# lhoyer/improving_segmentation_with_selfsupervised_depth

Hardware: AMD Instinct MI355X
Metric: train images/sec, ResNet-101 joint seg+depth @512x1024 (higher is better)
Workload: dtype f32

## Files before the change

### improving_segmentation_with_selfsupervised_depth_amd/csrc/conv_igemm.hip

```cpp
#include <type_traits>
#include "segsde_common.h"
#include "conv_small.h"
#include "winograd.h"
#include <cstdlib>
#include <mutex>
#include <cstring>

namespace {

struct ConvP {
  const float* x0; const float* x1; const float* w; const float* bias;
  float* y; float* y2;
  int B, H, W, C0, C1, ld0, ld1, up0;
  int Ho, Wo, N, ldy, ldy2, nsplit;
  int KH, KW, stride, dil, pad, pad_mode, in_div;
  int Ctot, Ktot, M, act, sum2x2;
  int vecout;
  int nb, ne;
  const float* zero;
  int kh0, khs, kw0, kws, KWf, Kfull, os, oph, opw, OHf, OWf;
  double* stats;
  int accum;
  const float* agy; int agld, agkind;
  unsigned mg1, mg2; int sf1, sf2, d1, d2;
// ... 1621 lines not shown
    return (b.ne - b.nb <= 32) ? launch_igemm<128, 32, 4, 1>(b, s) : launch_igemm<128, 64, 2, 2>(b, s);
  }
  return launch_igemm<128, 128, 2, 2>(q, s);
}

__global__ __launch_bounds__(256) void adjoint_corner_kernel(const float* dy, int lddy, const float* wd , float* y, int ldy,
                                                             float* y2, int ldy2, int nsplit, int B, int H, int W, int N, int C,
                                                             const float* agy, int agld, int agkind, int accumulate_only) {
  const int total = B * 4 * N;
  for (int e = blockIdx.x * 256 + threadIdx.x; e < total; e += gridDim.x * 256) {
    const int n = e % N, t = e / N, k = t & 3, b = t >> 2;
    const int bot = k >> 1, rgt = k & 1;
    const int i = bot ? H - 2 : 1, j = rgt ? W - 2 : 1, r = bot ? H - 1 : 0, sc = rgt ? W - 1 : 0;
    const int tap = (bot ? 0 : 2) * 3 + (rgt ? 0 : 2);
    const float* dp = dy + ((long)(b * H + r) * W + sc) * lddy;
    const float* wp = wd + ((long)n * 9 + tap) * C;
    float acc = 0.f;
    for (int c = 0; c < C; ++c) acc += dp[c] * wp[c];
    const long pix = (long)(b * H + i) * W + j;
    if (agy && n < nsplit) acc *= segsde_act_grad_from_out(agy[pix * agld + n], agkind);
    if (n < nsplit) y[pix * ldy + n] += acc; else y2[pix * ldy2 + (n - nsplit)] += acc;
  }
}

int launch_adjoint_by_borders(const ConvP& p, hipStream_t s, bool with_main = true) {
  ConvP q = p;
  q.pad_mode = SEGSDE_PAD_ZERO;
  ConvP bl[4];
  for (int k = 0; k < 4; ++k) {
    const bool rowl = k < 2, far = k & 1;
    ConvP b = p;
    b.pad_mode = SEGSDE_PAD_ZERO;
    b.KH = rowl ? 1 : 3; b.KW = rowl ? 3 : 1;
    b.Ho = rowl ? 1 : p.H; b.Wo = rowl ? p.W : 1; b.M = p.B * b.Ho * b.Wo;
    b.pad = rowl ? (far ? -(p.H - 1) : 0) : 1;
    b.padw = rowl ? 1 : (far ? -(p.W - 1) : 0);
    b.Ktot = 3 * p.Ctot; b.Kfull = p.Kfull; b.KWf = b.KW;
    b.wtap = rowl ? p.Ctot : 3 * p.Ctot;
    const int tap0 = rowl ? (far ? 0 : 6) : (far ? 0 : 2);
    b.w = p.w + (long)tap0 * p.Ctot;
    b.kh0 = 0; b.khs = 1; b.kw0 = 0; b.kws = 1;
    b.submap = 1; b.os = 1; b.OHf = p.H; b.OWf = p.W;
    b.oph = rowl ? (far ? p.H - 2 : 1) : 0; b.opw = rowl ? 0 : (far ? p.W - 2 : 1);
    b.osfast = (rowl && p.W % 128 == 0) ? 1 : 0;
    b.accum = 1; b.lin = 0; b.stats = nullptr; b.bias = nullptr; b.act = 0;
    set_divs(b);
    if (!igemm_fast_ok(b) || !b.vecout) return SEGSDE_ERR_UNSUPPORTED;
    bl[k] = b;
  }
  if (with_main)
    if (int e = launch_by_n(q, s)) return e;
  for (int k = 0; k < 4; ++k)
    if (int e = launch_by_n(bl[k], s)) return e;
  if (probing()) return 0;
  hipLaunchKernelGGL(adjoint_corner_kernel, dim3(segsde_cdiv((long)p.B * 4 * p.N, 256)), dim3(256), 0, s, p.x0, p.ld0, p.w, p.y, p.ldy,
                     p.y2, p.ldy2, p.nsplit, p.B, p.H, p.W, p.N, p.Ctot, p.agy, p.agld, p.agkind, 0);
  SEGSDE_CHECK_LAUNCH();
  return 0;
}
bool adjoint_by_borders_ok(const ConvP& p) {
  const bool big = (long)p.B * p.H * p.W >= (1L << 21) || p.cmp;
  return big && p.pad_mode == SEGSDE_PAD_REFLECT_ADJOINT && igemm_fast_ok(p) && !p.sum2x2 && p.vecout && p.H >= 4 &&
         p.W >= 4 && p.C1 == 0 && p.KH == 3 && p.KW == 3 && p.nb == 0 && p.ne == p.N;
}
}

namespace {
int borders_params(const segsde_conv_desc* d, const float* dy, const float* wdpack, float* y, const float* act_out, int act_ld,
                   int act_kind, ConvP& p) {
  if (int e = validate(d)) return e;
  if (d->pad_mode != SEGSDE_PAD_REFLECT_ADJOINT || d->C1 || d->up0 || d->sum2x2 || d->in_div > 1 || d->act != 0) return SEGSDE_ERR_UNSUPPORTED;
  p = make_params(d, dy, nullptr, wdpack, nullptr, y, nullptr);
  if (act_out) {
    if (act_kind < SEGSDE_ACT_RELU || act_kind > SEGSDE_ACT_SIGMOID || act_ld < p.nsplit || (act_ld % 4) || !aligned16(act_out))
      return SEGSDE_ERR_UNSUPPORTED;
    p.agy = act_out; p.agld = act_ld; p.agkind = act_kind;
  }
  if (!(igemm_fast_ok(p) && p.vecout && p.H >= 4 && p.W >= 4 && p.KH == 3 && p.KW == 3 && p.nb == 0 && p.ne == p.N))
    return SEGSDE_ERR_UNSUPPORTED;
  return 0;
}
}

extern "C" int segsde_reflect_adjoint_borders_ok(const segsde_conv_desc* d, int act_ld) {
  ConvP p;
  float* fake = reinterpret_cast<float*>(16);
  return borders_params(d, fake, fake, fake, act_ld ? fake : nullptr, act_ld, SEGSDE_ACT_ELU, p) == 0;
}

extern "C" int segsde_reflect_adjoint_borders(const segsde_conv_desc* d, const float* dy, const float* wdpack, float* y,
                                              const float* act_out, int act_ld, int act_kind, void* stream) {
  if (!dy || !wdpack || !y) return SEGSDE_ERR_NULL;
  ConvP p;
  if (int e = borders_params(d, dy, wdpack, y, act_out, act_ld, act_kind, p)) return e;
  return launch_adjoint_by_borders(p, static_cast<hipStream_t>(stream), false);
}

extern "C" long segsde_conv2d_stats_rows(const segsde_conv_desc* d) {
  if (validate(d)) return 0;
  float dummy[4];
  const ConvP p = make_params(d, dummy, dummy, dummy, nullptr, reinterpret_cast<float*>(16), nullptr);
  return stats_rows(d, p);
}

extern "C" int segsde_conv2d_forward(const segsde_conv_desc* d, const float* x0, const float* x1, const float* wpack,
                                     const float* bias, float* y, float* y2, void* stream) {
  return segsde_conv2d_forward_stats(d, x0, x1, wpack, bias, y, y2, nullptr, stream);
}

extern "C" int segsde_conv2d_forward_stats(const segsde_conv_desc* d, const float* x0, const float* x1, const float* wpack,
                                           const float* bias, float* y, float* y2, double* stats, void* stream) {
  return segsde_conv2d_dgrad_actgrad(d, x0, x1, wpack, bias, y, y2, stats, nullptr, 0, 0, stream);
}

extern "C" int segsde_conv2d_dgrad_actgrad(const segsde_conv_desc* d, const float* x0, const float* x1, const float* wpack,
                                           const float* bias, float* y, float* y2, double* stats, const float* act_out,
                                           int act_ld, int act_kind, void* stream) {
  if (int e = validate(d)) return e;
  if (!x0 || !wpack || !y || (d->C1 && !x1)) return SEGSDE_ERR_NULL;
  ConvP p = make_params(d, x0, x1, wpack, bias, y, y2);
  if (act_out) {
    if (stats || bias || d->act != 0 || act_kind < SEGSDE_ACT_RELU || act_kind > SEGSDE_ACT_SIGMOID || act_ld < p.nsplit ||
        (act_ld % 4) || !aligned16(act_out) || d->in_div > 1)
      return SEGSDE_ERR_UNSUPPORTED;
    p.agy = act_out; p.agld = act_ld; p.agkind = act_kind;
  }
  if (stats) {
    if (stats_rows(d, p) == 0) return SEGSDE_ERR_UNSUPPORTED;
    p.stats = stats;
  }
  const bool parity_split = d->in_div == 2 && d->stride == 1 && (d->dil & 1) && d->pad_mode == SEGSDE_PAD_ZERO && !d->sum2x2 &&
                            d->C1 == 0 && !d->up0 && !bias && d->act == 0 && !y2 && p.vecout;
  if (d->accumulate) {
    if (y2 || bias || d->act != 0 || d->sum2x2 || (d->in_div > 1 && !parity_split) || !p.vecout || d->Cout == 1 || d->C0 % 4 != 0 ||
        d->C0 == 1 || (d->pad_mode == SEGSDE_PAD_REFLECT_ADJOINT && !igemm_fast_ok(p)))
      return SEGSDE_ERR_UNSUPPORTED;
  }
  hipStream_t s = static_cast<hipStream_t>(stream);
  const bool plain3x3 = d->KH == 3 && d->KW == 3 && d->stride == 1 && d->dil == 1 && d->pad == 1 && d->C1 == 0 && !d->up0 &&
                        d->in_div <= 1 && !d->sum2x2 && d->H == d->Ho && d->W == d->Wo;
  if (plain3x3 && d->Cout == 1 && d->pad_mode != SEGSDE_PAD_REFLECT_ADJOINT && segsde_c1_supported(d->C0, d->ld0) &&
      aligned16(x0) && aligned16(wpack))
    return probing() ? 0 : segsde_c1_forward(x0, d->ld0, d->B, d->H, d->W, d->C0, wpack, bias, d->pad_mode == SEGSDE_PAD_REFLECT, d->act, y,
                             d->ldy, stream);
  if (plain3x3 && d->C0 == 1 && d->pad_mode != SEGSDE_PAD_REFLECT && !bias && d->act == 0 &&
      segsde_c1_supported(d->Cout, p.ldy) && p.vecout)
    return probing() ? 0 : segsde_c1_dgrad(x0, d->ld0, d->B, d->H, d->W, d->Cout, wpack, d->pad_mode == SEGSDE_PAD_REFLECT_ADJOINT, y, p.ldy,
                           y2, p.ldy2, p.nsplit, p.agy, p.agld, p.agkind, stream);
  const bool plain1x1 = d->KH == 1 && d->KW == 1 && d->stride == 1 && d->pad == 0 && d->C1 == 0 && !d->up0 && d->in_div <= 1 &&
                        !d->sum2x2 && d->H == d->Ho && d->W == d->Wo;
  if (plain1x1 && !stats && !p.agy && d->C0 % 4 != 0 && d->ld0 == d->C0 && aligned16(x0) && !bias && d->act == 0 && !y2 &&
      segsde_skinny_supported(d->C0, d->Cout) && p.vecout)
    return probing() ? 0 : segsde_skinny_nk(x0, d->C0, wpack, (long)d->B * d->H * d->W, d->Cout, y, p.ldy, stream);
  if (parity_split) {
    bool ok = true;
    ConvP sub[4]; int nsub = 0; bool empty = false;
    for (int ph = 0; ph < 2 && ok; ++ph)
      for (int pw = 0; pw < 2 && ok; ++pw) {
        ConvP q = p;
        int kh0 = -1, kw0 = -1;
        for (int k = 0; k < d->KH; ++k) if (((ph + k * d->dil - d->pad) & 1) == 0) { kh0 = k; break; }
        for (int k = 0; k < d->KW; ++k) if (((pw + k * d->dil - d->pad) & 1) == 0) { kw0 = k; break; }
        const int nI = (d->Ho - ph + 1) / 2, nJ = (d->Wo - pw + 1) / 2;
        if (nI <= 0 || nJ <= 0) continue;
        if (kh0 < 0 || kw0 < 0) { empty = true; continue; }
        q.kh0 = kh0; q.khs = 2; q.kw0 = kw0; q.kws = 2; q.KWf = d->KW; q.Kfull = p.Ktot;
        q.KH = (d->KH - kh0 + 1) / 2; q.KW = (d->KW - kw0 + 1) / 2;
        q.Ktot = q.KH * q.KW * q.Ctot;
        q.in_div = 1;
        q.pad = -((ph + kh0 * d->dil - d->pad) / 2);
        q.padw = -((pw + kw0 * d->dil - d->pad) / 2);
        q.os = 2; q.submap = 1; q.oph = ph; q.opw = pw; q.OHf = d->Ho; q.OWf = d->Wo;
        q.Ho = nI; q.Wo = nJ; q.M = d->B * nI * nJ;
        set_divs(q);
        if (!igemm_fast_ok(q)) ok = false;
        sub[nsub++] = q;
      }
    if (!ok && d->accumulate) return SEGSDE_ERR_UNSUPPORTED;
    if (ok) {
      if (empty && !d->accumulate && !probing()) {
        if (hipMemsetAsync(y, 0, (size_t)d->B * d->Ho * d->Wo * p.ldy * sizeof(float), s) != hipSuccess) return SEGSDE_ERR_SHAPE;
      }
      for (int i = 0; i < nsub; ++i) {
        const ConvP& q = sub[i];
        int e;
        if (q.N <= 32) e = launch_igemm<128, 32, 4, 1>(q, s);
        else if (q.N <= 64) e = launch_igemm<128, 64, 2, 2>(q, s);
        else e = launch_igemm<128, 128, 2, 2>(q, s);
        if (e) return e;
      }
      return 0;
    }
  }
  if (p.agy && d->pad_mode == SEGSDE_PAD_REFLECT_ADJOINT && !igemm_fast_ok(p))
    return SEGSDE_ERR_UNSUPPORTED;
  if (d->sum2x2) {
    if ((d->Ho & 1) || (d->Wo & 1) || d->stride != 1 || d->act != 0 || bias) return SEGSDE_ERR_SHAPE;
    if (!igemm_fast_ok(p)) return SEGSDE_ERR_UNSUPPORTED;
  }
  if (adjoint_by_borders_ok(p)) {
    const int e = launch_adjoint_by_borders(p, s);
    if (e != SEGSDE_ERR_UNSUPPORTED) return e;
  }
  if (int e = launch_by_n(p, s)) return e;
  if (d->pad_mode == SEGSDE_PAD_REFLECT_ADJOINT && !igemm_fast_ok(p))
    return launch_reflect_fix(x0, p.ld0, wpack, y, p.ldy, y2, p.ldy2, p.nsplit, p.B, p.H, p.W, p.N, p.C0, s);
  return 0;
}

namespace {
template <int BKT, int BN, int WM, int WN, int MODE, int CMP = 0>
int launch_wgrad_mode(const ConvP& p, const float* dy, int lddy, float* ws, int splits, int cps, hipStream_t stream) {
  const dim3 grid(segsde_cdiv(p.Ktot, BKT) * segsde_cdiv(p.N, BN) * splits);
  size_t smem = 2 * (size_t)BP * (BKT + BN) * sizeof(float);
  if (MODE == 5)
    smem += 2 * (size_t)((p.Ho - 1) * p.stride + (p.KH - 1) * p.dil + 1 + (p.Wo - 1) * p.stride + (p.KW - 1) * p.dil + 1) * sizeof(unsigned);
  auto k = conv_wgrad_kernel<BKT, BN, WM, WN, MODE, CMP>;
  (void)hipFuncSetAttribute(reinterpret_cast<const void*>(k), hipFuncAttributeMaxDynamicSharedMemorySize, (int)smem);
  hipLaunchKernelGGL(k, grid, dim3(256), smem, stream, p, dy, lddy, ws, cps);
  SEGSDE_CHECK_LAUNCH();
  return 0;
}

int wgrad_mode(const ConvP& p, const float* dy, int lddy) {
  const bool vec = vec_ok(p) && (p.N % 4 == 0) && (lddy % 4 == 0) && aligned16(dy);
  const long e0 = (long)p.B * (p.H >> p.up0) * (p.W >> p.up0) * p.ld0, e1 = (long)p.B * p.H * p.W * p.ld1;
  const bool fast = vec_ok(p) && e0 < (1L << 31) && e1 < (1L << 31);
  const long i0 = (long)(p.H >> p.up0) * (p.W >> p.up0) * p.ld0 * 4, i1 = (long)p.H * p.W * p.ld1 * 4;
  const bool table = p.Wo % BP == 0 && i0 <= (1L << 30) && i1 <= (1L << 30) && (long)BP * p.os * lddy * 4 < (1L << 30);
  if (fast && vec && table) return 5;
  if (fast) return 3;
  return vec ? 1 : 0;
}

int wgrad_compute(const ConvP& p, const float* dy, int lddy) { return wgrad_mode(p, dy, lddy) == 5 ? p.cmp : 0; }

template <int BKT, int BN, int WM, int WN>
int launch_wgrad(const ConvP& p, const float* dy, int lddy, float* ws, int splits, int cps, hipStream_t stream) {
  const int cmp = wgrad_compute(p, dy, lddy);
  if (probing()) return probe_note(cmp);
  switch (wgrad_mode(p, dy, lddy)) {
    case 5:
      return cmp == 1   ? launch_wgrad_mode<BKT, BN, WM, WN, 5, 1>(p, dy, lddy, ws, splits, cps, stream)
             : cmp == 2 ? launch_wgrad_mode<BKT, BN, WM, WN, 5, 2>(p, dy, lddy, ws, splits, cps, stream)
                        : launch_wgrad_mode<BKT, BN, WM, WN, 5, 0>(p, dy, lddy, ws, splits, cps, stream);
    case 3: return launch_wgrad_mode<BKT, BN, WM, WN, 3>(p, dy, lddy, ws, splits, cps, stream);
    case 1: return launch_wgrad_mode<BKT, BN, WM, WN, 1>(p, dy, lddy, ws, splits, cps, stream);
    default: return launch_wgrad_mode<BKT, BN, WM, WN, 0>(p, dy, lddy, ws, splits, cps, stream);
  }
}

void wgrad_plan(const segsde_conv_desc* d, int& bkt, int& bn, int& splits, int& cps) {
  const int Ktot = d->KH * d->KW * (d->C0 + d->C1);
  const long M = (long)d->B * d->Ho * d->Wo;
  bn = d->Cout <= 32 ? 32 : (d->Cout <= 64 ? 64 : 128);
  bkt = 128;
  const long tiles = (long)segsde_cdiv(Ktot, bkt) * segsde_cdiv(d->Cout, bn);
  const int nchunks = segsde_cdiv(M, BP);
  const long slots = 256L * (bn == 128 ? 2 : 3);
  constexpr long WG_OVERHEAD_CHUNKS = 4;
  long best = -1, best_cost = 0;
  const long smax = nchunks / 8 > 1 ? (nchunks / 8 < 1024 ? nchunks / 8 : 1024) : 1;
  for (long sp = 1; sp <= smax; ++sp) {
    const long c = (nchunks + sp - 1) / sp, se = (nchunks + c - 1) / c;
    const long waves = (tiles * se + slots - 1) / slots;
    const long cost = waves * (c + WG_OVERHEAD_CHUNKS);
    if (best < 0 || cost < best_cost) { best = se; best_cost = cost; }
  }
  cps = segsde_cdiv(nchunks, best);
  splits = segsde_cdiv(nchunks, cps);
}
}

namespace {
bool c1_wgrad_route(const segsde_conv_desc* d) {
  return d->Cout == 1 && d->KH == 3 && d->KW == 3 && d->stride == 1 && d->dil == 1 && d->pad == 1 && d->C1 == 0 && !d->up0 &&
         d->H == d->Ho && d->W == d->Wo && d->pad_mode != SEGSDE_PAD_REFLECT_ADJOINT && segsde_c1_supported(d->C0, d->ld0);
}
}

extern "C" size_t segsde_conv2d_wgrad_workspace(const segsde_conv_desc* d) {
  if (validate(d)) return 0;
  if (c1_wgrad_route(d)) return segsde_c1_wgrad_workspace(d->C0);
  int bkt, bn, splits, cps;
  wgrad_plan(d, bkt, bn, splits, cps);
  return (size_t)splits * d->KH * d->KW * (d->C0 + d->C1) * d->Cout * sizeof(float);
}

extern "C" int segsde_conv2d_wgrad(const segsde_conv_desc* d, const float* x0, const float* x1, const float* dy,
                                   int lddy, float* dw_oihw, float* workspace, size_t workspace_bytes, void* stream) {
  if (int e = validate(d)) return e;
  if (!x0 || !dy || !dw_oihw || !workspace || (d->C1 && !x1)) return SEGSDE_ERR_NULL;
  if (workspace_bytes < segsde_conv2d_wgrad_workspace(d)) return SEGSDE_ERR_WORKSPACE;
  if (c1_wgrad_route(d) && aligned16(x0))
    return probing() ? 0 : segsde_c1_wgrad(x0, d->ld0, d->B, d->H, d->W, d->C0, dy, lddy, d->pad_mode == SEGSDE_PAD_REFLECT, dw_oihw, workspace,
                           stream);
  ConvP p = make_params(d, x0, x1, dy , nullptr, workspace, nullptr);
  hipStream_t s = static_cast<hipStream_t>(stream);
  int bkt, bn, splits, cps;
  wgrad_plan(d, bkt, bn, splits, cps);
  int e;
  if (bn == 32) e = launch_wgrad<128, 32, 4, 1>(p, dy, lddy, workspace, splits, cps, s);
  else if (bn == 64) e = launch_wgrad<128, 64, 2, 2>(p, dy, lddy, workspace, splits, cps, s);
  else e = launch_wgrad<128, 128, 2, 2>(p, dy, lddy, workspace, splits, cps, s);
  if (e) return e;
  if (probing()) return 0;
  const long total = (long)p.Ktot * p.N;
  hipLaunchKernelGGL(wgrad_reduce_kernel, dim3(segsde_cdiv(total, 32)), dim3(256), 1024, s, workspace, splits,
                     p.Ktot, p.N, p.Ctot, d->KH * d->KW, (wgrad_mode(p, dy, lddy) == 5 && p.C1 > 0) ? p.C0 : 0, dw_oihw, p.Ctot, 0);
  SEGSDE_CHECK_LAUNCH();
  return 0;
}

namespace {
__device__ __host__ inline int upfold_th(int py, int kh) { return py == 0 ? (kh == 0 ? 0 : 1) : (kh == 2 ? 1 : 0); }

__global__ __launch_bounds__(256) void upfold_pack_kernel(const float* w, int Cout, int C0, int Ctot, float* wf, float* wd) {
  const long total = 4L * Cout * 4 * C0;
  for (long e = blockIdx.x * 256L + threadIdx.x; e < total; e += (long)gridDim.x * 256) {
    const int c = (int)(e % C0); long t = e / C0;
    const int tw = (int)(t & 1), th = (int)((t >> 1) & 1); t >>= 2;
    const int n = (int)(t % Cout), cls = (int)(t / Cout);
    const int py = cls >> 1, px = cls & 1;
    const float* wp = w + ((long)n * Ctot + c) * 9;
    float sum = 0.f;
    for (int kh = 0; kh < 3; ++kh) {
      if (upfold_th(py, kh) != th) continue;
      float r = 0.f;
      for (int kw = 0; kw < 3; ++kw)
        if (upfold_th(px, kw) == tw) r += wp[kh * 3 + kw];
      sum += r;
    }
    wf[e] = sum;
    const int a = 3 - 2 * th - py, b = 3 - 2 * tw - px;
    wd[(((long)c * 4 + a) * 4 + b) * Cout + n] = sum;
  }
}

__global__ __launch_bounds__(256) void upfold_dgrad_fix_kernel(const float* dy, int lddy, const float* wf, float* dx, int lddx,
                                                               int B, int H2, int W2, int C0, int Cout, const float* agy,
                                                               int agld, int agkind) {
  const int nbord = H2 >= 2 ? 2 * W2 + 2 * (H2 - 2) : W2;
  const long total = (long)B * nbord * C0;
  const int H = 2 * H2, W = 2 * W2;
  for (long e = blockIdx.x * 256L + threadIdx.x; e < total; e += (long)gridDim.x * 256) {
    const int c = (int)(e % C0); long t = e / C0;
    const int q = (int)(t % nbord), b = (int)(t / nbord);
    int i, j;
    if (q < W2) { i = 0; j = q; }
    else if (q < 2 * W2) { i = H2 - 1; j = q - W2; }
    else { const int r = q - 2 * W2; i = 1 + (r >> 1); j = (r & 1) ? W2 - 1 : 0; }
    float acc = 0.f;
    for (int a = 0; a < 4; ++a) {
      const int rm = 2 * i - 1 + a;
      const int rx = (i == 0 && a == 3) ? 0 : ((i == H2 - 1 && a == 0) ? H - 1 : -1);
      const int py = (a & 1) ? 0 : 1, th = a >= 2 ? 0 : 1;
      for (int bb = 0; bb < 4; ++bb) {
        const int cm = 2 * j - 1 + bb;
        const int cx = (j == 0 && bb == 3) ? 0 : ((j == W2 - 1 && bb == 0) ? W - 1 : -1);
        if (rx < 0 && cx < 0) continue;
        const int px = (bb & 1) ? 0 : 1, tw = bb >= 2 ? 0 : 1;
        const float* wrow = wf + (((long)(py * 2 + px) * Cout) * 4 + th * 2 + tw) * C0 + c;
        for (int v = 0; v < 3; ++v) {
          const int r = v == 1 ? rm : rx, sc = v == 0 ? cm : cx;
          if (r < 0 || r >= H || sc < 0 || sc >= W) continue;
          const float* dp = dy + ((long)(b * H + r) * W + sc) * lddy;
          float part = 0.f;
          for (int n = 0; n < Cout; ++n) part += dp[n] * wrow[(long)n * 4 * C0];
          acc += part;
        }
      }
    }
    const long pix = (long)(b * H2 + i) * W2 + j;
    if (agy) acc *= segsde_act_grad_from_out(agy[pix * agld + c], agkind);
    dx[pix * lddx + c] += acc;
  }
}

__global__ __launch_bounds__(256) void upfold_dgrad_corner_kernel(const float* dy, int lddy, const float* wdfold, float* dx, int lddx,
                                                                  int B, int H2, int W2, int C0, int Cout, const float* agy,
                                                                  int agld, int agkind) {
  const int total = B * 4 * C0;
  const int H = 2 * H2, W = 2 * W2;
  for (int e = blockIdx.x * 256 + threadIdx.x; e < total; e += gridDim.x * 256) {
    const int c = e % C0, t = e / C0, k = t & 3, b = t >> 2;
    const int bot = k >> 1, rgt = k & 1;
    const int i = bot ? H2 - 1 : 0, j = rgt ? W2 - 1 : 0, r = bot ? H - 1 : 0, sc = rgt ? W - 1 : 0;
    const int a = bot ? 0 : 3, bb = rgt ? 0 : 3;
    const float* dp = dy + ((long)(b * H + r) * W + sc) * lddy;
    const float* wp = wdfold + (((long)c * 4 + a) * 4 + bb) * Cout;
    float acc = 0.f;
    for (int n = 0; n < Cout; ++n) acc += dp[n] * wp[n];
    const long pix = (long)(b * H2 + i) * W2 + j;
    if (agy) acc *= segsde_act_grad_from_out(agy[pix * agld + c], agkind);
    dx[pix * lddx + c] += acc;
  }
}

__global__ __launch_bounds__(256) void upfold_wgrad_reduce_kernel(const float* part, int splits, int C0, int N, float* dw,
                                                                  int CtotDst) {
  SEGSDE_SMEM;
  float* sh = reinterpret_cast<float*>(segsde_smem);
  const long total = (long)N * C0 * 9;
  const long slab = 4L * C0 * N;
  const int tx = threadIdx.x & 31, ty = threadIdx.x >> 5;
  const long e = blockIdx.x * 32L + tx;
  float acc = 0.f;
  int n = 0, tap = 0, c = 0;
  if (e < total) {
    n = (int)(e % N); const long t = e / N;
    tap = (int)(t % 9); c = (int)(t / 9);
    const int kh = tap / 3, kw = tap - kh * 3;
    for (int cls = 0; cls < 4; ++cls) {
      const int th = upfold_th(cls >> 1, kh), tw = upfold_th(cls & 1, kw);
      const float* src = part + (long)cls * splits * slab + ((long)(th * 2 + tw) * C0 + c) * N + n;
      float s0 = 0.f, s1 = 0.f;
      int z = ty;
      for (; z + 8 < splits; z += 16) { s0 += src[(long)z * slab]; s1 += src[(long)(z + 8) * slab]; }
      if (z < splits) s0 += src[(long)z * slab];
      acc += s0 + s1;
    }
  }
  sh[ty * 32 + tx] = acc;
  __syncthreads();
  if (ty == 0 && e < total) {
    float s = 0.f;
    for (int j = 0; j < 8; ++j) s += sh[j * 32 + tx];
    dw[((long)n * CtotDst + c) * 9 + tap] = s;
  }
}

bool upfold_shape_ok(const segsde_conv_desc* d) {
  return d->up0 && d->KH == 3 && d->KW == 3 && d->stride == 1 && d->dil == 1 && d->pad == 1 && d->pad_mode == SEGSDE_PAD_REFLECT &&
         d->H == d->Ho && d->W == d->Wo && !(d->H & 1) && !(d->W & 1) && d->H >= 4 && d->W >= 4 && d->C0 % 32 == 0 &&
         d->C1 % 32 == 0 && d->Cout % 4 == 0 && d->in_div <= 1 && !d->sum2x2 && !d->accumulate;
}

ConvP upfold_class_fwd(const segsde_conv_desc* d, const float* x0, const float* wf, const float* bias, float* y, int py, int px) {
  segsde_conv_desc c = *d;
  c.H = d->H / 2; c.W = d->W / 2; c.Ho = c.H; c.Wo = c.W; c.up0 = 0; c.C1 = 0; c.ld1 = 0; c.KH = 2; c.KW = 2;
  c.pad = 1 - py; c.pad_mode = SEGSDE_PAD_ZERO; c.nsplit = 0; c.ldy2 = 0;
  if (d->C1) c.act = 0;
  ConvP q = make_params(&c, x0, nullptr, wf + (long)(py * 2 + px) * d->Cout * 4 * d->C0, d->C1 ? nullptr : bias, y, nullptr);
  q.pad_mode = SEGSDE_PAD_CLAMP_; q.padw = 1 - px;
  q.os = 2; q.submap = 1; q.oph = py; q.opw = px; q.OHf = d->H; q.OWf = d->W;
  q.osfast = (c.Wo % 128 == 0) ? 1 : 0;
  q.lin = 0;
  return q;
}
// ... 545 lines not shown
```

### improving_segmentation_with_selfsupervised_depth_amd/csrc/conv_small.h

```cpp
#pragma once
#include <stddef.h>
bool segsde_c1_supported(int C, int ldx);
size_t segsde_c1_wgrad_workspace(int C);
int segsde_c1_forward(const float* x, int ldx, int B, int H, int W, int C, const float* wpack, const float* bias, int reflect,
                      int act, float* y, int ldy, void* stream);
int segsde_c1_dgrad(const float* dz, int lddz, int B, int H, int W, int C, const float* wdpack, int adjoint, float* dx, int lddx,
                    float* dx2, int lddx2, int nsplit, const float* agy, int agld, int agkind, void* stream);
int segsde_c1_wgrad(const float* x, int ldx, int B, int H, int W, int C, const float* dz, int lddz, int reflect, float* dw,
                    float* workspace, void* stream);
bool segsde_skinny_supported(int K, int C);
int segsde_skinny_nk(const float* a, int K, const float* w, long M, int C, float* y, int ldy, void* stream);
```

### improving_segmentation_with_selfsupervised_depth_amd/csrc/conv_small.hip

```cpp
#include "segsde_common.h"
#include "conv_small.h"

namespace {
#define ST(s) static_cast<hipStream_t>(s)

__device__ __forceinline__ int refl1(int i, int n) { return i < 0 ? -i : (i >= n ? 2 * n - 2 - i : i); }

template <int LP>
__global__ __launch_bounds__(256) void c1_fwd_kernel(const float* x, int ldx, int B, int H, int W, const float* wp ,
                                                     const float* bias, int reflect, int act, float* y, int ldy) {
  constexpr int PPB = 256 / LP;
  const int lane_c = threadIdx.x % LP, slot = threadIdx.x / LP;
  float4 w[9];
#pragma unroll
  for (int t = 0; t < 9; ++t) w[t] = *reinterpret_cast<const float4*>(wp + t * (LP * 4) + 4 * lane_c);
  const float b0 = bias ? bias[0] : 0.f;
  const long npix = (long)B * H * W;
  for (long p0 = (long)blockIdx.x * PPB; p0 < npix; p0 += (long)gridDim.x * PPB) {
    const long p = p0 + slot;
    const bool live = p < npix;
    const long pp = live ? p : 0;
    const int wq = (int)(pp % W); const long t2 = pp / W; const int hq = (int)(t2 % H); const long b = t2 / H;
    float acc = 0.f;
#pragma unroll
    for (int kh = 0; kh < 3; ++kh) {
      int hi = hq + kh - 1; bool okh = true;
      if (reflect) hi = refl1(hi, H); else okh = (unsigned)hi < (unsigned)H;
#pragma unroll
      for (int kw = 0; kw < 3; ++kw) {
        int wi = wq + kw - 1; bool ok = okh;
        if (reflect) wi = refl1(wi, W); else ok = ok && (unsigned)wi < (unsigned)W;
        if (ok) {
          const float4 v = *reinterpret_cast<const float4*>(x + ((b * H + hi) * W + wi) * ldx + 4 * lane_c);
          const float4 ww = w[kh * 3 + kw];
          acc += v.x * ww.x + v.y * ww.y + v.z * ww.z + v.w * ww.w;
        }
      }
    }
#pragma unroll
    for (int o = LP / 2; o > 0; o >>= 1) acc += __shfl_xor(acc, o);
    if (lane_c == 0 && live) y[p * ldy] = segsde_act(acc + b0, act);
  }
}

template <int LP>
__global__ __launch_bounds__(256) void c1_dgrad_kernel(const float* dz, int lddz, int B, int H, int W,
                                                       const float* wd , int adjoint, float* dx, int lddx,
                                                       float* dx2, int lddx2, int nsplit, const float* agy, int agld,
                                                       int agkind) {
  constexpr int PPB = 256 / LP;
  const int lane_c = threadIdx.x % LP, slot = threadIdx.x / LP;
  float w[4][9];
#pragma unroll
  for (int j = 0; j < 4; ++j)
#pragma unroll
    for (int t = 0; t < 9; ++t) w[j][t] = wd[(4 * lane_c + j) * 9 + t];
  const long npix = (long)B * H * W;
  for (long p0 = (long)blockIdx.x * PPB; p0 < npix; p0 += (long)gridDim.x * PPB) {
    const long p = p0 + slot;
    if (p >= npix) continue;
    const int wq = (int)(p % W); const long t2 = p / W; const int hq = (int)(t2 % H); const long b = t2 / H;
    float a0 = 0.f, a1 = 0.f, a2 = 0.f, a3 = 0.f;
    int hp[3], wpp[3], nh = 0, nw = 0;
    hp[nh++] = hq; wpp[nw++] = wq;
    if (adjoint) {
      if (hq == 1) hp[nh++] = -1;
      if (hq == H - 2) hp[nh++] = H;
      if (wq == 1) wpp[nw++] = -1;
      if (wq == W - 2) wpp[nw++] = W;
    }
    for (int a = 0; a < nh; ++a)
      for (int bb = 0; bb < nw; ++bb)
#pragma unroll
        for (int kh = 0; kh < 3; ++kh) {
          const int yh = hp[a] + kh - 1;
          if ((unsigned)yh >= (unsigned)H) continue;
#pragma unroll
          for (int kw = 0; kw < 3; ++kw) {
            const int yw = wpp[bb] + kw - 1;
            if ((unsigned)yw >= (unsigned)W) continue;
            const float g = dz[((b * H + yh) * W + yw) * lddz];
            const int t = kh * 3 + kw;
            a0 += g * w[0][t]; a1 += g * w[1][t]; a2 += g * w[2][t]; a3 += g * w[3][t];
          }
        }
    const int c = 4 * lane_c;
    float* dst = c < nsplit ? dx + p * lddx + c : dx2 + p * lddx2 + (c - nsplit);
    if (agy && c < nsplit) {
      const float4 yv = *reinterpret_cast<const float4*>(agy + p * agld + c);
      a0 *= segsde_act_grad_from_out(yv.x, agkind); a1 *= segsde_act_grad_from_out(yv.y, agkind);
      a2 *= segsde_act_grad_from_out(yv.z, agkind); a3 *= segsde_act_grad_from_out(yv.w, agkind);
    }
    *reinterpret_cast<float4*>(dst) = make_float4(a0, a1, a2, a3);
  }
}

template <int LP>
__global__ __launch_bounds__(256) void c1_wgrad_kernel(const float* x, int ldx, int B, int H, int W, const float* dz,
                                                       int lddz, int reflect, float* part ) {
  constexpr int PPB = 256 / LP;
  SEGSDE_SMEM;
  float* sh = reinterpret_cast<float*>(segsde_smem);
  const int lane_c = threadIdx.x % LP, slot = threadIdx.x / LP;
  float4 acc[9];
#pragma unroll
  for (int t = 0; t < 9; ++t) acc[t] = make_float4(0.f, 0.f, 0.f, 0.f);
  const long npix = (long)B * H * W;
  for (long p0 = (long)blockIdx.x * PPB; p0 < npix; p0 += (long)gridDim.x * PPB) {
    const long p = p0 + slot;
    if (p >= npix) continue;
    const int wq = (int)(p % W); const long t2 = p / W; const int hq = (int)(t2 % H); const long b = t2 / H;
    const float g = dz[p * lddz];
#pragma unroll
    for (int kh = 0; kh < 3; ++kh) {
      int hi = hq + kh - 1; bool okh = true;
      if (reflect) hi = refl1(hi, H); else okh = (unsigned)hi < (unsigned)H;
#pragma unroll
      for (int kw = 0; kw < 3; ++kw) {
        int wi = wq + kw - 1; bool ok = okh;
        if (reflect) wi = refl1(wi, W); else ok = ok && (unsigned)wi < (unsigned)W;
        if (ok) {
          const float4 v = *reinterpret_cast<const float4*>(x + ((b * H + hi) * W + wi) * ldx + 4 * lane_c);
          float4& a = acc[kh * 3 + kw];
          a.x += v.x * g; a.y += v.y * g; a.z += v.z * g; a.w += v.w * g;
        }
      }
    }
  }
  constexpr int C = LP * 4;
#pragma unroll
  for (int t = 0; t < 9; ++t) *reinterpret_cast<float4*>(sh + (slot * 9 + t) * C + 4 * lane_c) = acc[t];
  __syncthreads();
  for (int e = threadIdx.x; e < 9 * C; e += 256) {
    float s = 0.f;
    for (int q = 0; q < PPB; ++q) s += sh[q * 9 * C + e];
    part[(long)blockIdx.x * 9 * C + e] = s;
  }
}

__global__ __launch_bounds__(256) void c1_wgrad_reduce_kernel(const float* part, int nblk, int C, float* dw ) {
  const int e = blockIdx.x * 16 + (threadIdx.x >> 4), l = threadIdx.x & 15;
  const bool live = e < 9 * C;
  float s4[4] = {0.f, 0.f, 0.f, 0.f};
  if (live)
    for (int z = l; z < nblk; z += 64) {
#pragma unroll
      for (int u = 0; u < 4; ++u)
        if (z + 16 * u < nblk) s4[u] += part[(long)(z + 16 * u) * 9 * C + e];
    }
  float s = (s4[0] + s4[1]) + (s4[2] + s4[3]);
#pragma unroll
  for (int d = 8; d > 0; d >>= 1) s += __shfl_xor(s, d);
  if (live && l == 0) {
    const int tap = e / C, c = e - tap * C;
// ... 114 lines not shown
  __syncthreads();
  for (int e = threadIdx.x; e < 9 * C; e += 256) {
    float s = 0.f;
    for (int q = 0; q < G; ++q) s += sh[q * 9 * C + e];
    part[(long)blockIdx.x * 9 * C + e] = s;
  }
}

template <int LP>
__global__ __launch_bounds__(256) void c1s_dgrad_kernel(const float* dz, int lddz, int B, int H, int W, const float* wd ,
                                                        int adjoint, float* dx, int lddx, float* dx2, int lddx2, int nsplit,
                                                        const float* agy, int agld, int agkind) {
  constexpr int G = 256 / LP;
  const int lane_c = threadIdx.x % LP, slot = threadIdx.x / LP;
  float w[4][9];
#pragma unroll
  for (int j = 0; j < 4; ++j)
#pragma unroll
    for (int t = 0; t < 9; ++t) w[j][t] = wd[(4 * lane_c + j) * 9 + t];
  const int c = 4 * lane_c;
  const int nsr = W / CS, nstrips = B * H * nsr;
  for (int s0 = blockIdx.x * G; s0 < nstrips; s0 += gridDim.x * G) {
    const Strip st = strip_decode(s0 + slot, nstrips, nsr, H);
    if (!st.live) continue;
    const size_t pix0 = (size_t)(st.b * H + st.h) * W + st.w0;
    float* dst = c < nsplit ? dx + pix0 * lddx + c : dx2 + pix0 * lddx2 + (c - nsplit);
    const int ldd = c < nsplit ? lddx : lddx2;
    const float* ag = (agy && c < nsplit) ? agy + pix0 * agld + c : nullptr;
    auto put = [&](int o, float a0, float a1, float a2, float a3) {
      if (ag) {
        const float4 yv = *reinterpret_cast<const float4*>(ag + (size_t)o * agld);
        a0 *= segsde_act_grad_from_out(yv.x, agkind); a1 *= segsde_act_grad_from_out(yv.y, agkind);
        a2 *= segsde_act_grad_from_out(yv.z, agkind); a3 *= segsde_act_grad_from_out(yv.w, agkind);
      }
      *reinterpret_cast<float4*>(dst + (size_t)o * ldd) = make_float4(a0, a1, a2, a3);
    };
    const bool border = adjoint && (st.h == 1 || st.h == H - 2);
    const bool colfirst = adjoint && st.w0 == 0, collast = adjoint && st.w0 + CS == W;
    if (!border) {
      float4 yv[CS];
      if (ag) {
#pragma unroll
        for (int o = 0; o < CS; ++o) yv[o] = *reinterpret_cast<const float4*>(ag + (size_t)o * agld);
      }
      float g[3][CS + 2];
#pragma unroll
      for (int r = 0; r < 3; ++r) {
        const int yh = st.h + r - 1;
        const bool okh = (unsigned)yh < (unsigned)H;
        const float* gp = dz + (size_t)(st.b * H + (okh ? yh : 0)) * W * lddz;
#pragma unroll
        for (int j = 0; j < CS + 2; ++j) {
          const int yw = st.w0 - 1 + j;
          const bool ok = okh && (unsigned)yw < (unsigned)W;
          g[r][j] = 0.f;
          if (ok) g[r][j] = gp[(size_t)yw * lddz];
        }
      }
#pragma unroll
      for (int o = 0; o < CS; ++o) {
        float a0 = 0.f, a1 = 0.f, a2 = 0.f, a3 = 0.f;
#pragma unroll
        for (int kh = 0; kh < 3; ++kh)
#pragma unroll
          for (int kw = 0; kw < 3; ++kw) {
            const float gv = g[kh][o + kw];
            const int t = kh * 3 + kw;
            a0 += gv * w[0][t]; a1 += gv * w[1][t]; a2 += gv * w[2][t]; a3 += gv * w[3][t];
          }
        if ((colfirst && o == 1) || (collast && o == CS - 2)) {
          const int j = o == 1 ? 1 : CS, kw = o == 1 ? 2 : 0;
#pragma unroll
          for (int kh = 0; kh < 3; ++kh) {
            const float gv = g[kh][j];
            const int t = kh * 3 + kw;
            a0 += gv * w[0][t]; a1 += gv * w[1][t]; a2 += gv * w[2][t]; a3 += gv * w[3][t];
          }
        }
        if (ag) {
          a0 *= segsde_act_grad_from_out(yv[o].x, agkind); a1 *= segsde_act_grad_from_out(yv[o].y, agkind);
          a2 *= segsde_act_grad_from_out(yv[o].z, agkind); a3 *= segsde_act_grad_from_out(yv[o].w, agkind);
        }
        *reinterpret_cast<float4*>(dst + (size_t)o * ldd) = make_float4(a0, a1, a2, a3);
      }
    } else {
      for (int o = 0; o < CS; ++o) {
        const int hq = st.h, wq = st.w0 + o;
        float a0 = 0.f, a1 = 0.f, a2 = 0.f, a3 = 0.f;
        int hp[3], wpp[3], nh = 0, nw = 0;
        hp[nh++] = hq; wpp[nw++] = wq;
        if (hq == 1) hp[nh++] = -1;
        if (hq == H - 2) hp[nh++] = H;
        if (wq == 1) wpp[nw++] = -1;
        if (wq == W - 2) wpp[nw++] = W;
        for (int a = 0; a < nh; ++a)
          for (int bb = 0; bb < nw; ++bb)
#pragma unroll
            for (int kh = 0; kh < 3; ++kh) {
              const int yh = hp[a] + kh - 1;
              if ((unsigned)yh >= (unsigned)H) continue;
#pragma unroll
              for (int kw = 0; kw < 3; ++kw) {
                const int yw = wpp[bb] + kw - 1;
                if ((unsigned)yw >= (unsigned)W) continue;
                const float gv = dz[((size_t)(st.b * H + yh) * W + yw) * lddz];
                const int t = kh * 3 + kw;
                a0 += gv * w[0][t]; a1 += gv * w[1][t]; a2 += gv * w[2][t]; a3 += gv * w[3][t];
              }
            }
        put(o, a0, a1, a2, a3);
      }
    }
  }
}

constexpr int SKP = 64;

__device__ __forceinline__ void skinny_stage(const float* src, long p0, int n, int K, float* sh) {
  const float* base = src + p0 * K;
  const int total = n * K, t4 = total & ~3;
  for (int e = threadIdx.x * 4; e < t4; e += 1024) *reinterpret_cast<float4*>(sh + e) = *reinterpret_cast<const float4*>(base + e);
  for (int e = t4 + threadIdx.x; e < total; e += 256) sh[e] = base[e];
}

template <int LP, int KB>
__global__ __launch_bounds__(256) void skinny_nk_kernel(const float* a, int K, const float* w, long M, float* y, int ldy) {
  constexpr int G = 256 / LP;
  SEGSDE_SMEM;
  float* sh = reinterpret_cast<float*>(segsde_smem);
  const int lane_c = threadIdx.x % LP, slot = threadIdx.x / LP;
  float wr[KB][4];
#pragma unroll
  for (int k = 0; k < KB; ++k)
#pragma unroll
    for (int j = 0; j < 4; ++j) wr[k][j] = k < K ? w[(long)(4 * lane_c + j) * K + k] : 0.f;
  for (long p0 = (long)blockIdx.x * SKP; p0 < M; p0 += (long)gridDim.x * SKP) {
    const int n = (int)(M - p0 < SKP ? M - p0 : SKP);
    __syncthreads();
    skinny_stage(a, p0, n, K, sh);
    __syncthreads();
    for (int q = slot; q < n; q += G) {
      const float* gp = sh + q * K;
      float a0 = 0.f, a1 = 0.f, a2 = 0.f, a3 = 0.f;
#pragma unroll
      for (int k = 0; k < KB; ++k) {
        const float g = k < K ? gp[k] : 0.f;
        a0 += g * wr[k][0]; a1 += g * wr[k][1]; a2 += g * wr[k][2]; a3 += g * wr[k][3];
      }
      *reinterpret_cast<float4*>(y + (p0 + q) * ldy + 4 * lane_c) = make_float4(a0, a1, a2, a3);
    }
  }
}

inline int c1_blocks(long npix, int ppb) { long nb = (npix + ppb - 1) / ppb; return (int)(nb < 1 ? 1 : (nb > 2048 ? 2048 : nb)); }
}

bool segsde_c1_supported(int C, int ldx) { return (C == 64 || C == 128 || C == 256) && (ldx % 4 == 0); }

size_t segsde_c1_wgrad_workspace(int C) { return (size_t)1024 * 9 * C * sizeof(float); }

inline int c1s_blocks(int B, int H, int W, int groups) {
  const long nb = ((long)B * H * (W / CS) + groups - 1) / groups;
  return (int)(nb < 1 ? 1 : (nb > 4096 ? 4096 : nb));
}
inline bool c1_strips(int B, int H, int W) { return W % CS == 0 && (long)B * H * W < (1L << 31); }

#define C1_DISPATCH(KERNEL, grid, smem, ...)                                                       \
  do {                                                                                             \
    if (C == 64) hipLaunchKernelGGL((KERNEL<16>), grid, dim3(256), smem, ST(stream), __VA_ARGS__);  \
    else if (C == 128) hipLaunchKernelGGL((KERNEL<32>), grid, dim3(256), smem, ST(stream), __VA_ARGS__); \
    else hipLaunchKernelGGL((KERNEL<64>), grid, dim3(256), smem, ST(stream), __VA_ARGS__);          \
  } while (0)

int segsde_c1_forward(const float* x, int ldx, int B, int H, int W, int C, const float* wpack, const float* bias, int reflect,
                      int act, float* y, int ldy, void* stream) {
  if (c1_strips(B, H, W)) {
    const dim3 grid(c1s_blocks(B, H, W, 256 / (C / 4)));
    C1_DISPATCH(c1s_fwd_kernel, grid, 0, x, ldx, B, H, W, wpack, bias, reflect, act, y, ldy);
    SEGSDE_CHECK_LAUNCH();
    return 0;
  }
  const dim3 grid(c1_blocks((long)B * H * W, 256 / (C / 4)));
  C1_DISPATCH(c1_fwd_kernel, grid, 0, x, ldx, B, H, W, wpack, bias, reflect, act, y, ldy);
  SEGSDE_CHECK_LAUNCH();
  return 0;
}

int segsde_c1_dgrad(const float* dz, int lddz, int B, int H, int W, int C, const float* wdpack, int adjoint, float* dx, int lddx,
                    float* dx2, int lddx2, int nsplit, const float* agy, int agld, int agkind, void* stream) {
  if (!dx2) { dx2 = dx; lddx2 = lddx; nsplit = C; }
  if (c1_strips(B, H, W) && H >= 4 && W >= 2 * CS) {
    const dim3 grid(c1s_blocks(B, H, W, 256 / (C / 4)));
    C1_DISPATCH(c1s_dgrad_kernel, grid, 0, dz, lddz, B, H, W, wdpack, adjoint, dx, lddx, dx2, lddx2, nsplit, agy, agld, agkind);
    SEGSDE_CHECK_LAUNCH();
    return 0;
  }
  const dim3 grid(c1_blocks((long)B * H * W, 256 / (C / 4)));
  C1_DISPATCH(c1_dgrad_kernel, grid, 0, dz, lddz, B, H, W, wdpack, adjoint, dx, lddx, dx2, lddx2, nsplit, agy, agld, agkind);
  SEGSDE_CHECK_LAUNCH();
  return 0;
}

int segsde_c1_wgrad(const float* x, int ldx, int B, int H, int W, int C, const float* dz, int lddz, int reflect, float* dw,
                    float* workspace, void* stream) {
  const int ppb = 256 / (C / 4);
  long nb = ((long)B * H * W + ppb - 1) / ppb;
  const int nblk = (int)(nb < 1 ? 1 : (nb > 1024 ? 1024 : nb));
  const size_t smem = (size_t)ppb * 9 * C * sizeof(float);
  if (c1_strips(B, H, W)) {
    long ns = ((long)B * H * (W / CS) + ppb - 1) / ppb;
    const int nbs = (int)(ns < 1 ? 1 : (ns > 1024 ? 1024 : ns));
    C1_DISPATCH(c1s_wgrad_kernel, dim3(nbs), smem, x, ldx, B, H, W, dz, lddz, reflect, workspace);
    SEGSDE_CHECK_LAUNCH();
    hipLaunchKernelGGL(c1_wgrad_reduce_kernel, dim3((9 * C + 15) / 16), dim3(256), 0, ST(stream), (const float*)workspace, nbs,
                       C, dw);
    SEGSDE_CHECK_LAUNCH();
    return 0;
  }
  C1_DISPATCH(c1_wgrad_kernel, dim3(nblk), smem, x, ldx, B, H, W, dz, lddz, reflect, workspace);
  SEGSDE_CHECK_LAUNCH();
  hipLaunchKernelGGL(c1_wgrad_reduce_kernel, dim3((9 * C + 15) / 16), dim3(256), 0, ST(stream), (const float*)workspace, nblk,
                     C, dw);
  SEGSDE_CHECK_LAUNCH();
  return 0;
}

bool segsde_skinny_supported(int K, int C) { return K >= 1 && K <= 32 && (C == 64 || C == 128 || C == 256); }

#define SK_DISPATCH(KERNEL, grid, smem, ...)                                                                    \
  do {                                                                                                          \
    if (K <= 20) {                                                                                              \
      if (C == 64) hipLaunchKernelGGL((KERNEL<16, 20>), grid, dim3(256), smem, ST(stream), __VA_ARGS__);         \
      else if (C == 128) hipLaunchKernelGGL((KERNEL<32, 20>), grid, dim3(256), smem, ST(stream), __VA_ARGS__);   \
      else hipLaunchKernelGGL((KERNEL<64, 20>), grid, dim3(256), smem, ST(stream), __VA_ARGS__);                 \
    } else {                                                                                                    \
      if (C == 64) hipLaunchKernelGGL((KERNEL<16, 32>), grid, dim3(256), smem, ST(stream), __VA_ARGS__);         \
      else if (C == 128) hipLaunchKernelGGL((KERNEL<32, 32>), grid, dim3(256), smem, ST(stream), __VA_ARGS__);   \
      else hipLaunchKernelGGL((KERNEL<64, 32>), grid, dim3(256), smem, ST(stream), __VA_ARGS__);                 \
    }                                                                                                           \
  } while (0)

int segsde_skinny_nk(const float* a, int K, const float* w, long M, int C, float* y, int ldy, void* stream) {
  long nb = (M + SKP - 1) / SKP;
  const dim3 grid((unsigned)(nb < 1 ? 1 : (nb > 8192 ? 8192 : nb)));
  SK_DISPATCH(skinny_nk_kernel, grid, (size_t)SKP * 32 * sizeof(float), a, K, w, M, y, ldy);
  SEGSDE_CHECK_LAUNCH();
  return 0;
}
```

Baseline: 62.37.

## Add specialized skinny 1x1 conv forward and weight-gradient kernels for small Cout

Adds dedicated kernels for 1x1 convolutions with few output channels (Cout up to 32, such as segmentation and depth heads). The forward kernel stages input rows in shared memory, keeps weight and bias in registers and writes outputs with a fused activation. The weight-gradient kernel accumulates per-block partial outer products over pixels, then a separate reduction kernel sums them. Both are meant to replace the general implicit-GEMM path, whose tiles are badly shaped for tiny N. The cost is extra workspace and a two-pass reduction, and the new paths can be switched off through environment variables.

```diff
diff --git a/improving_segmentation_with_selfsupervised_depth_amd/csrc/conv_igemm.hip b/improving_segmentation_with_selfsupervised_depth_amd/csrc/conv_igemm.hip
--- a/improving_segmentation_with_selfsupervised_depth_amd/csrc/conv_igemm.hip
+++ b/improving_segmentation_with_selfsupervised_depth_amd/csrc/conv_igemm.hip
@@ -1797,6 +1797,9 @@
   if (plain1x1 && !stats && !p.agy && d->C0 % 4 != 0 && d->ld0 == d->C0 && aligned16(x0) && !bias && d->act == 0 && !y2 &&
       segsde_skinny_supported(d->C0, d->Cout) && p.vecout)
     return probing() ? 0 : segsde_skinny_nk(x0, d->C0, wpack, (long)d->B * d->H * d->W, d->Cout, y, p.ldy, stream);
+  if (plain1x1 && !stats && !p.agy && !y2 && !d->accumulate && d->compute == 0 && d->Cout <= 32 && aligned16(x0) && aligned16(wpack) &&
+      segsde_skinny_kn_supported(d->Cout, d->C0, d->ld0))
+    return probing() ? 0 : segsde_skinny_kn(x0, d->ld0, wpack, bias, d->Cout, d->act, (long)d->B * d->H * d->W, d->C0, y, d->ldy, stream);
   if (parity_split) {
     bool ok = true;
     ConvP sub[4]; int nsub = 0; bool empty = false;
@@ -1918,6 +1921,10 @@
 }
 
 namespace {
+bool skinny_wgrad_route(const segsde_conv_desc* d) {
+  return d->KH == 1 && d->KW == 1 && d->stride == 1 && d->pad == 0 && d->C1 == 0 && !d->up0 && d->H == d->Ho && d->W == d->Wo &&
+         d->compute == 0 && d->Cout <= 32 && segsde_skinny_wgrad_supported(d->Cout, d->C0, d->ld0);
+}
 bool c1_wgrad_route(const segsde_conv_desc* d) {
   return d->Cout == 1 && d->KH == 3 && d->KW == 3 && d->stride == 1 && d->dil == 1 && d->pad == 1 && d->C1 == 0 && !d->up0 &&
          d->H == d->Ho && d->W == d->Wo && d->pad_mode != SEGSDE_PAD_REFLECT_ADJOINT && segsde_c1_supported(d->C0, d->ld0);
@@ -1929,7 +1936,12 @@
   if (c1_wgrad_route(d)) return segsde_c1_wgrad_workspace(d->C0);
   int bkt, bn, splits, cps;
   wgrad_plan(d, bkt, bn, splits, cps);
-  return (size_t)splits * d->KH * d->KW * (d->C0 + d->C1) * d->Cout * sizeof(float);
+  const size_t slabs = (size_t)splits * d->KH * d->KW * (d->C0 + d->C1) * d->Cout * sizeof(float);
+  if (skinny_wgrad_route(d)) {
+    const size_t sk = segsde_skinny_wgrad_workspace(d->Cout, d->C0);
+    return sk > slabs ? sk : slabs;
+  }
+  return slabs;
 }
 
 extern "C" int segsde_conv2d_wgrad(const segsde_conv_desc* d, const float* x0, const float* x1, const float* dy,
@@ -1940,6 +1952,8 @@
   if (c1_wgrad_route(d) && aligned16(x0))
     return probing() ? 0 : segsde_c1_wgrad(x0, d->ld0, d->B, d->H, d->W, d->C0, dy, lddy, d->pad_mode == SEGSDE_PAD_REFLECT, dw_oihw, workspace,
                            stream);
+  if (skinny_wgrad_route(d) && lddy == d->Cout && aligned16(x0))
+    return probing() ? 0 : segsde_skinny_wgrad(x0, d->ld0, dy, d->Cout, (long)d->B * d->H * d->W, d->C0, dw_oihw, workspace, stream);
   ConvP p = make_params(d, x0, x1, dy , nullptr, workspace, nullptr);
   hipStream_t s = static_cast<hipStream_t>(stream);
   int bkt, bn, splits, cps;
diff --git a/improving_segmentation_with_selfsupervised_depth_amd/csrc/conv_small.h b/improving_segmentation_with_selfsupervised_depth_amd/csrc/conv_small.h
--- a/improving_segmentation_with_selfsupervised_depth_amd/csrc/conv_small.h
+++ b/improving_segmentation_with_selfsupervised_depth_amd/csrc/conv_small.h
@@ -10,3 +10,9 @@
                     float* workspace, void* stream);
 bool segsde_skinny_supported(int K, int C);
 int segsde_skinny_nk(const float* a, int K, const float* w, long M, int C, float* y, int ldy, void* stream);
+bool segsde_skinny_kn_supported(int K, int C, int ldx);
+int segsde_skinny_kn(const float* x, int ldx, const float* w, const float* bias, int K, int act, long M, int C, float* y, int ldy,
+                     void* stream);
+bool segsde_skinny_wgrad_supported(int K, int C, int ldx);
+size_t segsde_skinny_wgrad_workspace(int K, int C);
+int segsde_skinny_wgrad(const float* x, int ldx, const float* dy, int K, long M, int C, float* dw, float* workspace, void* stream);
diff --git a/improving_segmentation_with_selfsupervised_depth_amd/csrc/conv_small.hip b/improving_segmentation_with_selfsupervised_depth_amd/csrc/conv_small.hip
--- a/improving_segmentation_with_selfsupervised_depth_amd/csrc/conv_small.hip
+++ b/improving_segmentation_with_selfsupervised_depth_amd/csrc/conv_small.hip
@@ -1,5 +1,6 @@
 #include "segsde_common.h"
 #include "conv_small.h"
+#include <stdlib.h>
 
 namespace {
 #define ST(s) static_cast<hipStream_t>(s)
@@ -420,6 +421,196 @@
   }
 }
 
+
+template <int C, int KO>
+__global__ __launch_bounds__(256) void skinny_kn_kernel(const float* __restrict__ x, int ldx, const float* __restrict__ w ,
+                                                        const float* __restrict__ bias, int K, int act, long M,
+                                                        float* __restrict__ y, int ldy) {
+  constexpr int ROW = C + 4, C4 = C / 4;
+  constexpr int NV = SKP * C4 / 256;
+  constexpr int NE = SKP * 4 * KO / 256;
+  SEGSDE_SMEM;
+  float* shx = reinterpret_cast<float*>(segsde_smem);
+  float* sho = shx + SKP * ROW;
+  const int KS = K | 1;
+  const int pix = threadIdx.x & 63;
+  const int j = __builtin_amdgcn_readfirstlane((int)(threadIdx.x >> 6));
+  int so[NE], go[NE];
+#pragma unroll
+  for (int i = 0; i < NE; ++i) {
+    const int e = threadIdx.x + i * 256, q = e / K, k = e - q * K;
+    so[i] = q * KS + k; go[i] = q * ldy + k;
+  }
+  float bk[KO];
+  const float4* wk[KO];
+#pragma unroll
+  for (int o = 0; o < KO; ++o) {
+    const int k = j * KO + o, kk = k < K ? k : K - 1;
+    bk[o] = bias ? bias[kk] : 0.f;
+    wk[o] = reinterpret_cast<const float4*>(w + (long)kk * C);
+  }
+  float4 pre[NV];
+  auto fetch = [&](long p0) {
+    const long n = M - p0;
+#pragma unroll
+    for (int i = 0; i < NV; ++i) {
+      const int e = threadIdx.x + i * 256, q = e / C4, c4 = e - q * C4;
+      pre[i] = make_float4(0.f, 0.f, 0.f, 0.f);
+      if (q < n) pre[i] = *reinterpret_cast<const float4*>(x + (p0 + q) * ldx + 4 * c4);
+    }
+  };
+  const long step = (long)gridDim.x * SKP;
+  long p0 = (long)blockIdx.x * SKP;
+  if (p0 < M) fetch(p0);
+  for (; p0 < M; p0 += step) {
+    const int n = (int)(M - p0 < SKP ? M - p0 : SKP);
+    __syncthreads();
+#pragma unroll
+    for (int i = 0; i < NV; ++i) {
+      const int e = threadIdx.x + i * 256, q = e / C4, c4 = e - q * C4;
+      *reinterpret_cast<float4*>(shx + q * ROW + 4 * c4) = pre[i];
+    }
+    __syncthreads();
+    if (p0 + step < M) fetch(p0 + step);
+    float acc[KO];
+#pragma unroll
+    for (int o = 0; o < KO; ++o) acc[o] = 0.f;
+    const float4* xr = reinterpret_cast<const float4*>(shx + pix * ROW);
+#pragma unroll 4
+    for (int c4 = 0; c4 < C4; ++c4) {
+      const float4 v = xr[c4];
+#pragma unroll
+      for (int o = 0; o < KO; ++o) {
+        const float4 ww = wk[o][c4];
+        acc[o] = fmaf(v.w, ww.w, fmaf(v.z, ww.z, fmaf(v.y, ww.y, fmaf(v.x, ww.x, acc[o]))));
+      }
+    }
+#pragma unroll
+    for (int o = 0; o < KO; ++o) {
+      const int k = j * KO + o;
+      if (k < K) sho[pix * KS + k] = segsde_act(acc[o] + bk[o], act);
+    }
+    __syncthreads();
+    float* yp = y + p0 * ldy;
+#pragma unroll
+    for (int i = 0; i < NE; ++i)
+      if ((int)threadIdx.x + i * 256 < n * K) yp[go[i]] = sho[so[i]];
+  }
+}
+
+template <int LP, int KB>
+__global__ __launch_bounds__(256, KB <= 20 ? 3 : 1) void skinny_wgrad_kernel(const float* __restrict__ x, int ldx, const float* __restrict__ dy ,
+                                                           int K, long M, float* __restrict__ part ) {
+  constexpr int G = 256 / LP, C = 4 * LP, U = 4, RP = G * U, R = SKP / RP;
+  constexpr int NE = SKP * KB / 256;
+  static_assert(R >= 1 && KB % 4 == 0, "stage geometry");
+  SEGSDE_SMEM;
+  float* sh = reinterpret_cast<float*>(segsde_smem);
+  const int lane_c = threadIdx.x % LP, slot = threadIdx.x / LP;
+  float4 acc[KB];
+#pragma unroll
+  for (int k = 0; k < KB; ++k) acc[k] = make_float4(0.f, 0.f, 0.f, 0.f);
+  int so[NE];
+#pragma unroll
+  for (int i = 0; i < NE; ++i) {
+    const int e = threadIdx.x + i * 256, q = e / K;
+    so[i] = q * KB + (e - q * K);
+  }
+  for (int e = threadIdx.x; e < SKP * KB; e += 256) sh[e] = 0.f;
+  float dyr[NE];
+  auto fetch_dy = [&](long p0) {
+    const long n = (M - p0) * K;
+#pragma unroll
+    for (int i = 0; i < NE; ++i) {
+      const int e = threadIdx.x + i * 256;
+      dyr[i] = e < n && e < SKP * K ? dy[p0 * K + e] : 0.f;
+    }
+  };
+  auto fetch_x = [&](long pb, float4* v) {
+#pragma unroll
+    for (int u = 0; u < U; ++u) {
+      const long p = pb + u * G + slot;
+      v[u] = make_float4(0.f, 0.f, 0.f, 0.f);
+      if (p < M) v[u] = *reinterpret_cast<const float4*>(x + p * ldx + 4 * lane_c);
+    }
+  };
+  const long step = (long)gridDim.x * SKP;
+  long p0 = (long)blockIdx.x * SKP;
+  float4 xc[U], xn[U];
+  if (p0 < M) { fetch_dy(p0); fetch_x(p0, xc); }
+  for (; p0 < M; p0 += step) {
+    __syncthreads();
+#pragma unroll
+    for (int i = 0; i < NE; ++i)
+      if ((int)threadIdx.x + i * 256 < SKP * K) sh[so[i]] = dyr[i];
+    __syncthreads();
+    if (p0 + step < M) fetch_dy(p0 + step);
+#pragma unroll
+    for (int r = 0; r < R; ++r) {
+      fetch_x(r + 1 < R ? p0 + (r + 1) * RP : p0 + step, xn);
+#pragma unroll
+      for (int u = 0; u < U; ++u) {
+        const int q = r * RP + u * G + slot;
+        if (p0 + q < M) {
+          const float4* gp = reinterpret_cast<const float4*>(sh + q * KB);
+#pragma unroll
+          for (int k4 = 0; k4 < KB / 4; ++k4) {
+            const float4 g = gp[k4];
+            const float gg[4] = {g.x, g.y, g.z, g.w};
+#pragma unroll
+            for (int i = 0; i < 4; ++i) {
+              float4& a = acc[4 * k4 + i];
+              a.x = fmaf(gg[i], xc[u].x, a.x); a.y = fmaf(gg[i], xc[u].y, a.y);
+              a.z = fmaf(gg[i], xc[u].z, a.z); a.w = fmaf(gg[i], xc[u].w, a.w);
+            }
+          }
+        }
+      }
+#pragma unroll
+      for (int u = 0; u < U; ++u) xc[u] = xn[u];
+    }
+  }
+#pragma unroll
+  for (int k = 0; k < KB; ++k)
+#pragma unroll
+    for (int d = LP; d < 64; d <<= 1) {
+      acc[k].x += __shfl_xor(acc[k].x, d); acc[k].y += __shfl_xor(acc[k].y, d);
+      acc[k].z += __shfl_xor(acc[k].z, d); acc[k].w += __shfl_xor(acc[k].w, d);
+    }
+  const int wave = threadIdx.x >> 6, lane = threadIdx.x & 63;
+  float* dst = part + (long)blockIdx.x * K * C;
+#pragma unroll
+  for (int kc = 0; kc < KB / 4; ++kc) {
+    __syncthreads();
+    if (lane < LP) {
+#pragma unroll
+      for (int i = 0; i < 4; ++i) *reinterpret_cast<float4*>(sh + (wave * 4 + i) * C + 4 * lane) = acc[4 * kc + i];
+    }
+    __syncthreads();
+    for (int e = threadIdx.x; e < 4 * C; e += 256) {
+      const int k = 4 * kc + e / C;
+      const float s = ((sh[e] + sh[4 * C + e]) + sh[8 * C + e]) + sh[12 * C + e];
+      if (k < K) dst[(long)kc * 4 * C + e] = s;
+    }
+  }
+}
+
+__global__ __launch_bounds__(256) void skinny_wgrad_reduce_kernel(const float* part, int nblk, int n , float* dw) {
+  const int e = blockIdx.x * 16 + (threadIdx.x >> 4), l = threadIdx.x & 15;
+  const bool live = e < n;
+  float s4[4] = {0.f, 0.f, 0.f, 0.f};
+  if (live)
+    for (int z = l; z < nblk; z += 64) {
+#pragma unroll
+      for (int u = 0; u < 4; ++u)
+        if (z + 16 * u < nblk) s4[u] += part[(long)(z + 16 * u) * n + e];
+    }
+  float s = (s4[0] + s4[1]) + (s4[2] + s4[3]);
+#pragma unroll
+  for (int d = 8; d > 0; d >>= 1) s += __shfl_xor(s, d);
+  if (live && l == 0) dw[e] = s;
+}
+
 inline int c1_blocks(long npix, int ppb) { long nb = (npix + ppb - 1) / ppb; return (int)(nb < 1 ? 1 : (nb > 2048 ? 2048 : nb)); }
 }
 
@@ -515,3 +706,49 @@
   SEGSDE_CHECK_LAUNCH();
   return 0;
 }
+
+static bool env_on(const char* name) { const char* e = getenv(name); return !(e && e[0] == '0'); }
+
+bool segsde_skinny_kn_supported(int K, int C, int ldx) { return segsde_skinny_supported(K, C) && ldx % 4 == 0 && env_on("SEGSDE_SKINNY_FWD"); }
+
+int segsde_skinny_kn(const float* x, int ldx, const float* w, const float* bias, int K, int act, long M, int C, float* y, int ldy,
+                     void* stream) {
+  long nb = (M + SKP - 1) / SKP;
+  const dim3 grid((unsigned)(nb < 1 ? 1 : (nb > 2048 ? 2048 : nb)));
+  const size_t smem = ((size_t)SKP * (C + 4) + (size_t)SKP * (K | 1)) * sizeof(float);
+#define SKF_LAUNCH(CC, KO)                                                                                               \
+  do {                                                                                                                   \
+    auto k = skinny_kn_kernel<CC, KO>;                                                                                   \
+    (void)hipFuncSetAttribute(reinterpret_cast<const void*>(k), hipFuncAttributeMaxDynamicSharedMemorySize, (int)smem);  \
+    hipLaunchKernelGGL(k, grid, dim3(256), smem, ST(stream), x, ldx, w, bias, K, act, M, y, ldy);                        \
+  } while (0)
+  if (K <= 20) {
+    if (C == 64) SKF_LAUNCH(64, 5); else if (C == 128) SKF_LAUNCH(128, 5); else SKF_LAUNCH(256, 5);
+  } else {
+    if (C == 64) SKF_LAUNCH(64, 8); else if (C == 128) SKF_LAUNCH(128, 8); else SKF_LAUNCH(256, 8);
+  }
+#undef SKF_LAUNCH
+  SEGSDE_CHECK_LAUNCH();
+  return 0;
+}
+
+bool segsde_skinny_wgrad_supported(int K, int C, int ldx) { return segsde_skinny_supported(K, C) && ldx % 4 == 0 && env_on("SEGSDE_SKINNY_WGRAD"); }
+
+static int skinny_wgrad_blocks(int K, long M) {
+  const long nb = (M + SKP - 1) / SKP, cap = K <= 20 ? 768 : 256;
+  return (int)(nb < 1 ? 1 : (nb > cap ? cap : nb));
+}
+
+size_t segsde_skinny_wgrad_workspace(int K, int C) { return (size_t)768 * K * C * sizeof(float); }
+
+int segsde_skinny_wgrad(const float* x, int ldx, const float* dy, int K, long M, int C, float* dw, float* workspace, void* stream) {
+  const int nblk = skinny_wgrad_blocks(K, M);
+  const dim3 grid(nblk);
+  const int kb = K <= 20 ? 20 : 32;
+  const size_t smem = (size_t)(SKP * kb > 16 * C ? SKP * kb : 16 * C) * sizeof(float);
+  SK_DISPATCH(skinny_wgrad_kernel, grid, smem, x, ldx, dy, K, M, workspace);
+  SEGSDE_CHECK_LAUNCH();
+  hipLaunchKernelGGL(skinny_wgrad_reduce_kernel, dim3((K * C + 15) / 16), dim3(256), 0, ST(stream), (const float*)workspace, nblk, K * C, dw);
+  SEGSDE_CHECK_LAUNCH();
+  return 0;
+}
```

Result: no change. 62.54 (median of 6 runs) (+0.3%).
